# Dimitrinov74/Domain-Specific-Image-Compression

Hardware: AMD Instinct MI355X
Metric: 256x256 satellite patches encoded/s per GPU; bpp + MS-SSIM vs reference (higher is better)
Workload: dtype f32 (Winograd contractions as split-bf16 MFMA with fp32 accumulate); 1 GPU; batch=64/GPU 256x256x3 synthetic patches, modelv2 encode->decode (g_a,h_a,round,h_s,Student-t/Gaussian rate,g_s) + bpp + MS-SSIM[.3,.5,.2] on GPU + CDF tables and range coder (z,y strings) on GPU [BASELINE config 3]; global_batch=64, parallelism=per-image sharding x1, one all-reduce of 4 fp64, weights=synthetic seed 1 (checkpoints absent from the reference)

## Files before the change

domain-specific-image-compression_amd/csrc/dsic_math.h:

```cpp
#pragma once
#include <stdint.h>

#if defined(__HIPCC__)
#define DM_HD __host__ __device__ inline
#else
#define DM_HD inline
#endif

namespace dsic {
namespace dm {

#define DM_LN2_HI 6.93147180369123816490e-01
#define DM_LN2_LO 1.90821492927058770002e-10
#define DM_INV_LN2 1.44269504088896338700e+00
#define DM_SQRT2 1.41421356237309514547e+00
#define DM_INV_SQRT_PI 5.64189583547756279280e-01
#define DM_HALF_LOG_2PI 9.18938533204672780563e-01

DM_HD double from_bits(uint64_t b) {
  union {
    uint64_t u;
    double d;
  } v;
  v.u = b;
// ... 12 lines not shown
  while (k > 1000) {
    x *= 8.98846567431157953865e+307;
    k -= 1023;
  }
  while (k < -1000) {
    x *= 2.22507385850720138309e-308;
    k += 1022;
  }
  return x * from_bits((uint64_t)(k + 1023) << 52);
}

DM_HD double exp(double x) {
  if (x != x) return x;
  if (x > 709.0) return from_bits(0x7FF0000000000000ULL);
  if (x < -745.0) return 0.0;
  const double t = x * DM_INV_LN2;
  const int k = (int)(t < 0 ? t - 0.5 : t + 0.5);
  const double r = (x - (double)k * DM_LN2_HI) - (double)k * DM_LN2_LO;
  double p = 1.0 / 87178291200.0;
  p = p * r + 1.0 / 6227020800.0;
  p = p * r + 1.0 / 479001600;
  p = p * r + 1.0 / 39916800;
  p = p * r + 1.0 / 3628800;
  p = p * r + 1.0 / 362880;
  p = p * r + 1.0 / 40320;
  p = p * r + 1.0 / 5040;
  p = p * r + 1.0 / 720;
  p = p * r + 1.0 / 120;
  p = p * r + 1.0 / 24;
  p = p * r + 1.0 / 6;
  p = p * r + 0.5;
  p = p * r + 1.0;
  p = p * r + 1.0;
  return scale2(p, k);
}

DM_HD double log(double x) {
  if (x != x || x < 0) return from_bits(0x7FF8000000000000ULL);
  if (x == 0) return from_bits(0xFFF0000000000000ULL);
  int e = 0;
  if (x < 2.22507385850720138309e-308) {
    x *= 4503599627370496.0;
    e = -52;
  }
  uint64_t bits = to_bits(x);
  e += (int)((bits >> 52) & 0x7FF) - 1023;
  double m = from_bits((bits & 0x000FFFFFFFFFFFFFULL) | 0x3FF0000000000000ULL);
  if (m > DM_SQRT2) {
    m = m * 0.5;
    e += 1;
  }
  const double f = m - 1.0;
  const double s = f / (2.0 + f);
  const double z = s * s;
  double p = 1.0 / 25;
  for (int n = 11; n >= 1; --n) p = p * z + 1.0 / (double)(2 * n + 1);
  p = p * z + 1.0;
  const double de = (double)e;
  return de * DM_LN2_HI + (2.0 * s * p + de * DM_LN2_LO);
}

DM_HD double lgamma(double x) {
  double acc = 1.0;
  while (x < 12.0) {
    acc = acc * x;
    x = x + 1.0;
  }
  const double xi = 1.0 / x, x2 = xi * xi;
  double ser = 1.0 / 156;
  ser = ser * x2 - 691.0 / 360360;
  ser = ser * x2 + 1.0 / 1188;
  ser = ser * x2 - 1.0 / 1680;
  ser = ser * x2 + 1.0 / 1260;
  ser = ser * x2 - 1.0 / 360;
  ser = ser * x2 + 1.0 / 12;
  const double st = (x - 0.5) * log(x) - x + DM_HALF_LOG_2PI + ser * xi;
  return st - log(acc);
}

DM_HD double erfc_pos(double u) {
  if (u < 1.5) {
    const double u2 = u * u;
    double term = u, sum = u;
    for (int n = 1; n < 200; ++n) {
      term = term * (2.0 * u2) / (double)(2 * n + 1);
      sum = sum + term;
      if (term < sum * 1e-17) break;
    }
    return 1.0 - 2.0 * DM_INV_SQRT_PI * exp(-u2) * sum;
  }
  double d = u;
  for (int n = 120; n >= 1; --n) d = u + (0.5 * (double)n) / d;
  return exp(-u * u) * DM_INV_SQRT_PI / d;
}

DM_HD double normal_cdf(double x) {
  const double u = x / DM_SQRT2;
  if (u >= 0) return 1.0 - 0.5 * erfc_pos(u);
  return 0.5 * erfc_pos(-u);
}

DM_HD double betacf(double a, double b, double x) {
  const double TINY = 1e-300;
  const double qab = a + b, qap = a + 1.0, qam = a - 1.0;
  double c = 1.0, d = 1.0 - qab * x / qap;
  if (d < TINY && d > -TINY) d = TINY;
  d = 1.0 / d;
  double h = d;
  for (int m = 1; m <= 400; ++m) {
    const double dm_ = (double)m, m2 = 2.0 * dm_;
    double aa = dm_ * (b - dm_) * x / ((qam + m2) * (a + m2));
    d = 1.0 + aa * d;
    if (d < TINY && d > -TINY) d = TINY;
    c = 1.0 + aa / c;
    if (c < TINY && c > -TINY) c = TINY;
    d = 1.0 / d;
    h = h * d * c;
    aa = -(a + dm_) * (qab + dm_) * x / ((a + m2) * (qap + m2));
    d = 1.0 + aa * d;
    if (d < TINY && d > -TINY) d = TINY;
    c = 1.0 + aa / c;
    if (c < TINY && c > -TINY) c = TINY;
    d = 1.0 / d;
    const double del = d * c;
    h = h * del;
    double dev = del - 1.0;
    if (dev < 0) dev = -dev;
    if (dev < 3e-16) break;
  }
  return h;
}

DM_HD double betainc(double a, double b, double x, double xc) {
  if (x <= 0.0) return 0.0;
  if (xc <= 0.0) return 1.0;
  const double lbeta = lgamma(a + b) - lgamma(a) - lgamma(b);
  const double front = exp(lbeta + a * log(x) + b * log(xc));
  if (x < (a + 1.0) / (a + b + 2.0)) return front * betacf(a, b, x) / a;
  return 1.0 - front * betacf(b, a, xc) / b;
}

DM_HD double student_t_tail(double t, double nu) {
  const double t2 = t * t;
  const double den = nu + t2;
  const double x = nu / den, xc = t2 / den;
  return 0.5 * betainc(0.5 * nu, 0.5, x, xc);
}

DM_HD double student_t_cdf(double t, double nu) {
  const double tail = student_t_tail(t, nu);
  return t > 0 ? 1.0 - tail : tail;
}


DM_HD double erf_pos(double u) {
  if (u < 1.5) {
    const double u2 = u * u;
    double term = u, sum = u;
    for (int n = 1; n < 200; ++n) {
      term = term * (2.0 * u2) / (double)(2 * n + 1);
      sum = sum + term;
      if (term < sum * 1e-17) break;
    }
    return 2.0 * DM_INV_SQRT_PI * exp(-u2) * sum;
  }
  if (u > 6.0) return 1.0;
  return 1.0 - erfc_pos(u);
}

DM_HD float erff_rn(float a) {
  const double u = (double)a;
  if (u != u) return a;
  return u < 0 ? -(float)erf_pos(-u) : (float)erf_pos(u);
}

DM_HD float gaussian_cdf_f32(float x) {
  const float a = x / 1.41421354f;
  const float e = erff_rn(a);
  const float s = 1.0f + e;
  return 0.5f * s;
}

DM_HD float sum_f32_torch(const float* p, int n) {
  float a0 = 0.0f, a1 = 0.0f, a2 = 0.0f, a3 = 0.0f;
  int i = 0;
  while (i + 16 <= n) {
    for (int j = 0; j < 16; ++j, ++i) a0 = a0 + p[i];
    a1 = a1 + a0;
    a0 = 0.0f;
    if ((i & 0xF0) == 0) {
      a2 = a2 + a1;
      a1 = 0.0f;
      if ((i & 0xF00) == 0) {
        a3 = a3 + a2;
        a2 = 0.0f;
      }
    }
  }
  for (; i < n; ++i) a0 = a0 + p[i];
  a0 = a0 + a1;
  a0 = a0 + a2;
  a0 = a0 + a3;
  return a0;
}

DM_HD void finish_table(const float* F, int L, uint16_t* out, float* pmf, uint16_t* raw) {
  for (int k = 0; k < L; ++k) {
    float p = F[k + 1] - F[k];
    if (p < 1e-12f) p = 1e-12f;
    pmf[k] = p;
  }
  const float total = sum_f32_torch(pmf, L);
  double cum = 0.0;
  uint32_t u16 = 0;
  for (int k = 0; k < L; ++k) {
    out[k] = (uint16_t)((uint32_t)(((uint64_t)u16 * (uint64_t)(65536 - L)) / 65535u) + (uint32_t)k);
    if (raw) raw[k] = (uint16_t)u16;
    const float q = pmf[k] / total;
    cum = cum + (double)q;
    float c = (float)cum;
    if (k == L - 1 && c < 1.0f) c = 1.0f;
    float sc = c * 65535.0f;
    if (sc < 0.0f) sc = 0.0f;
    if (sc > 65535.0f) sc = 65535.0f;
    u16 = (uint32_t)sc;
  }
  if (raw) raw[L] = (uint16_t)u16;
}

DM_HD float boundary_f32(int smin, int k) { return (float)(smin + k) - 0.5f; }
DM_HD float table_cdf_gauss(int smin, int k, float sigma) {
  return gaussian_cdf_f32(boundary_f32(smin, k) / sigma);
}
DM_HD float table_cdf_student(int smin, int k, float sigma, float nu) {
  return (float)student_t_cdf((double)boundary_f32(smin, k) / (double)sigma, (double)nu);
}

}
}
```

domain-specific-image-compression_amd/csrc/entropy.hip:

```cpp
#include "common.h"
#include "dsic_math.h"

#include <climits>

namespace dsic {

__global__ __launch_bounds__(256) void support_kernel(const float* __restrict__ y,
                                                      const float* __restrict__ z,
                                                      int* __restrict__ meta, int64_t ny, int64_t nz,
                                                      int tail) {
  __shared__ float red[2][4];
  __shared__ int bad_any;
  const int b = blockIdx.x;
  for (int which = 0; which < 2; ++which) {
    const float* p = which ? z + (size_t)b * nz : y + (size_t)b * ny;
    const int64_t n = which ? nz : ny;
    float mn = p[0], mx = p[0];
    bool bad = false;
    for (int64_t i = threadIdx.x; i < n; i += 256) {
      const float v = p[i];
      bad |= !(fabsf(v) < 1.0e9f);
      mn = fminf(mn, v);
      mx = fmaxf(mx, v);
    }
#pragma unroll
    for (int o = 32; o > 0; o >>= 1) {
      mn = fminf(mn, __shfl_down(mn, o, 64));
      mx = fmaxf(mx, __shfl_down(mx, o, 64));
    }
    if (threadIdx.x == 0) bad_any = 0;
    __syncthreads();
    if ((threadIdx.x & 63) == 0) {
      red[0][threadIdx.x >> 6] = mn;
      red[1][threadIdx.x >> 6] = mx;
    }
    if (__any(bad) && (threadIdx.x & 63) == 0) atomicOr(&bad_any, 1);
    __syncthreads();
    if (threadIdx.x == 0) {
      mn = fminf(fminf(red[0][0], red[0][1]), fminf(red[0][2], red[0][3]));
      mx = fmaxf(fmaxf(red[1][0], red[1][1]), fmaxf(red[1][2], red[1][3]));
      if (bad_any) {
        meta[4 * b + 2 * which] = 0;
        meta[4 * b + 2 * which + 1] = 0;
      } else {
        const int lo = (int)floorf(mn) - tail, hi = (int)ceilf(mx) + tail;
        meta[4 * b + 2 * which] = lo;
        meta[4 * b + 2 * which + 1] = hi - lo + 1;
      }
    }
    __syncthreads();
  }
}

__device__ __forceinline__ void finish_table_wave(float* F, int L, uint16_t* out, float* pmf, int lane) {
  for (int k = lane; k < L; k += 64) {
    float p = F[k + 1] - F[k];
    if (p < 1e-12f) p = 1e-12f;
    pmf[k] = p;
  }
  __builtin_amdgcn_s_waitcnt(0xc07f);
  __builtin_amdgcn_wave_barrier();
  const float total = dm::sum_f32_torch(pmf, L);
  double cum = 0.0;
  for (int base = 0; base < L; base += 64) {
    const int k = base + lane;
    const float q = k < L ? pmf[k] / total : 0.0f;
    const int n = L - base < 64 ? L - base : 64;
    float mine = 0.0f;
    for (int j = 0; j < n; ++j) {
      const float qj = __builtin_bit_cast(float, __builtin_amdgcn_readlane(__builtin_bit_cast(int, q), j));
      cum = cum + (double)qj;
      float c = (float)cum;
      if (base + j == L - 1 && c < 1.0f) c = 1.0f;
      if (j == lane) mine = c;
    }
    if (k < L) F[k] = mine;
  }
  __builtin_amdgcn_s_waitcnt(0xc07f);
  __builtin_amdgcn_wave_barrier();
  for (int k = lane; k < L; k += 64) {
    uint32_t u16 = 0;
    if (k > 0) {
      float sc = F[k - 1] * 65535.0f;
      if (sc < 0.0f) sc = 0.0f;
      if (sc > 65535.0f) sc = 65535.0f;
      u16 = (uint32_t)sc;
    }
    out[k] = (uint16_t)((u16 * (uint32_t)(65536 - L)) / 65535u + (uint32_t)k);
  }
}

template <bool STUDENT>
__global__ __launch_bounds__(256) void tables_kernel(const float* __restrict__ sigma,
                                                     const float* __restrict__ nu, int sb,
                                                     const int* __restrict__ meta, int meta_off,
                                                     uint16_t* __restrict__ tables, int C, int Lmax,
                                                     int ntables, int* __restrict__ err) {
  extern __shared__ float shm[];
  const int wave = threadIdx.x >> 6, lane = threadIdx.x & 63;
  const int tid = blockIdx.x * 4 + wave;
  if (tid >= ntables) return;
  const int b = tid / C, c = tid % C;
  const int smin = meta[4 * b + meta_off], L = meta[4 * b + meta_off + 1];
  if (L > Lmax || L < 1) {
    if (lane == 0) atomicOr(err, 1);
    return;
  }
  float* F = shm + (size_t)wave * (2 * Lmax + 1);
  float* pmf = F + Lmax + 1;
  const float sg = sigma[(size_t)b * sb + c];
  const float nv = STUDENT ? nu[(size_t)b * sb + c] : 0.0f;
  if (STUDENT && smin <= 0 && smin + L >= 1) {
    const int whi = smin + L > 1 - smin ? smin + L : 1 - smin;
    for (int w = 1 + lane; w <= whi; w += 64) {
      const double tail = dm::student_t_tail((double)((float)w - 0.5f) / (double)sg, (double)nv);
      if (w <= smin + L) F[w - smin] = (float)(1.0 - tail);
      if (1 - w >= smin) F[1 - w - smin] = (float)tail;
    }
  } else {
    for (int k = lane; k <= L; k += 64)
      F[k] = STUDENT ? dm::table_cdf_student(smin, k, sg, nv) : dm::table_cdf_gauss(smin, k, sg);
  }
  __builtin_amdgcn_s_waitcnt(0xc07f);
  __builtin_amdgcn_wave_barrier();
  finish_table_wave(F, L, tables + ((size_t)b * C + c) * Lmax, pmf, lane);
}

constexpr int ZT_IMGS = 16;

__global__ __launch_bounds__(256) void gauss_tables_kernel(const float* __restrict__ sigma,
                                                           const int* __restrict__ meta,
                                                           uint16_t* __restrict__ tables, int B, int C, int Lmax,
                                                           int rowmax, int* __restrict__ err) {
  extern __shared__ float shm[];
  __shared__ int ulo, uhi;
  const int wave = threadIdx.x >> 6, lane = threadIdx.x & 63;
  const int c = blockIdx.x, b0 = blockIdx.y * ZT_IMGS;
  const int b1 = B - b0 < ZT_IMGS ? B : b0 + ZT_IMGS;
  const float sg = sigma[c];
  if (wave == 0) {
    int lo = INT_MAX, hi = INT_MIN;
    if (b0 + lane < b1 && lane < ZT_IMGS) {
      const int smin = meta[4 * (b0 + lane) + 2], L = meta[4 * (b0 + lane) + 3];
      if (L >= 1 && L <= Lmax) {
        lo = smin;
        hi = smin + L;
      }
    }
#pragma unroll
    for (int o = 32; o > 0; o >>= 1) {
      lo = min(lo, __shfl_xor(lo, o, 64));
      hi = max(hi, __shfl_xor(hi, o, 64));
    }
    if (lane == 0) {
      ulo = lo;
      uhi = hi;
    }
  }
  __syncthreads();
  const int lo = ulo, hi = uhi;
  const bool shared_row = hi >= lo && (int64_t)hi - lo < (int64_t)rowmax;
  float* row = shm;
  if (shared_row)
    for (int u = lo + (int)threadIdx.x; u <= hi; u += 256) row[u - lo] = dm::table_cdf_gauss(u, 0, sg);
  __syncthreads();
  float* F = shm + rowmax + (size_t)wave * (2 * Lmax + 1);
  float* pmf = F + Lmax + 1;
  for (int b = b0 + wave; b < b1; b += 4) {
    const int smin = meta[4 * b + 2], L = meta[4 * b + 3];
    if (L > Lmax || L < 1) {
      if (lane == 0) atomicOr(err, 1);
      continue;
    }
    for (int k = lane; k <= L; k += 64) F[k] = shared_row ? row[smin + k - lo] : dm::table_cdf_gauss(smin, k, sg);
    __builtin_amdgcn_s_waitcnt(0xc07f);
    __builtin_amdgcn_wave_barrier();
    finish_table_wave(F, L, tables + ((size_t)b * C + c) * Lmax, pmf, lane);
    __builtin_amdgcn_s_waitcnt(0xc07f);
    __builtin_amdgcn_wave_barrier();
  }
}

__device__ __forceinline__ void put_bits(uint32_t* out32, int64_t cap_bits, int64_t off, uint32_t v,
                                         int len, int* overflow) {
  if (off + len > cap_bits) {
    *overflow = 1;
    return;
  }
  const int64_t w = off >> 5;
  const int s = (int)(off & 31), space = 32 - s;
  if (len <= space) {
    atomicOr(out32 + w, __builtin_bswap32(v << (space - len)));
  } else {
    const int rest = len - space;
    atomicOr(out32 + w, __builtin_bswap32(v >> rest));
    atomicOr(out32 + w + 1, __builtin_bswap32(v << (32 - rest)));
  }
}

__device__ __forceinline__ void put_ones(uint32_t* out32, int64_t cap_bits, int64_t off, uint32_t count,
                                         int* overflow) {
  while (count > 0) {
    const int len = count > 32 ? 32 : (int)count;
    put_bits(out32, cap_bits, off, len == 32 ? 0xFFFFFFFFu : ((1u << len) - 1u), len, overflow);
    off += len;
    count -= len;
  }
}

constexpr int PLACE_WIN = 512;
__device__ __forceinline__ void or_word(uint32_t* out32, uint32_t* win, int64_t wbase, int64_t w, uint32_t v) {
  const int64_t i = w - wbase;
  if (i >= 0 && i < PLACE_WIN) atomicOr(win + i, v);
  else atomicOr(out32 + w, v);
}

__device__ __forceinline__ void put_bits_w(uint32_t* out32, uint32_t* win, int64_t wbase, int64_t cap_bits,
                                           int64_t off, uint32_t v, int len, int* overflow) {
  if (off + len > cap_bits) {
    *overflow = 1;
    return;
  }
  const int64_t w = off >> 5;
  const int s = (int)(off & 31), space = 32 - s;
  if (len <= space) {
    or_word(out32, win, wbase, w, __builtin_bswap32(v << (space - len)));
  } else {
    const int rest = len - space;
    or_word(out32, win, wbase, w, __builtin_bswap32(v >> rest));
    or_word(out32, win, wbase, w + 1, __builtin_bswap32(v << (32 - rest)));
  }
}

__device__ __forceinline__ void put_ones_w(uint32_t* out32, uint32_t* win, int64_t wbase, int64_t cap_bits,
                                           int64_t off, uint32_t count, int* overflow) {
  while (count > 0) {
    const int len = count > 32 ? 32 : (int)count;
    put_bits_w(out32, win, wbase, cap_bits, off, len == 32 ? 0xFFFFFFFFu : ((1u << len) - 1u), len, overflow);
    off += len;
    count -= len;
  }
}

#ifndef ENC_SELECT
#define ENC_SELECT 1
#endif
template <int J>
__device__ __forceinline__ void wlane(uint32_t& rec, uint32_t v) {
  asm volatile("v_writelane_b32 %0, %1, %2" : "+v"(rec) : "s"(v), "n"(J));
}

template <int J>
__device__ __forceinline__ uint32_t rlane(uint32_t v) {
  uint32_t r;
  asm volatile("v_readlane_b32 %0, %1, %2" : "=s"(r) : "v"(v), "n"(J));
  return r;
}

template <int J>
__device__ __forceinline__ void enc_step(uint32_t& low, uint32_t& lowm1, uint32_t& span, uint32_t& cl,
                                         uint32_t& ch, uint32_t clo16, uint32_t chi16, uint32_t& rec_low,
                                         uint32_t& rec_high) {
  const uint32_t cl_next = J < 63 ? rlane<(J < 63 ? J + 1 : 63)>(clo16) : 0u;
  const uint32_t ch_next = J < 63 ? rlane<(J < 63 ? J + 1 : 63)>(chi16) : 0u;
  uint32_t lo_add, hi_add;
#if ENC_SELECT
  {
    const uint32_t ml = __umulhi(span, cl), mh = __umulhi(span, ch);
    lo_add = span ? ml : cl;
    hi_add = span ? mh : ch;
  }
#else
  if (__builtin_expect(span == 0u, 0)) {
    lo_add = cl;
    hi_add = ch;
  } else {
    lo_add = __umulhi(span, cl);
    hi_add = __umulhi(span, ch);
  }
#endif
  const uint32_t low1 = low + lo_add;
  const uint32_t high1 = lowm1 + hi_add;
  const uint32_t span1 = hi_add - lo_add;
  wlane<J>(rec_low, low1);
  wlane<J>(rec_high, high1);
  const int nb = __builtin_clz(low1 ^ high1);
  const uint32_t q2 = (high1 | ~low1) << 1;
  const int m = __builtin_clz(q2 << nb);
  const int sh = nb + m;
  span = span1 << sh;
  low = (low1 << sh) & 0x7FFFFFFFu;
  lowm1 = low - 1u;
  cl = cl_next;
  ch = ch_next;
}

template <int J0>
__device__ __forceinline__ void enc_steps8(uint32_t& low, uint32_t& lowm1, uint32_t& span, uint32_t& cl,
                                           uint32_t& ch, uint32_t clo16, uint32_t chi16, uint32_t& rec_low,
                                           uint32_t& rec_high) {
  enc_step<J0 + 0>(low, lowm1, span, cl, ch, clo16, chi16, rec_low, rec_high);
  enc_step<J0 + 1>(low, lowm1, span, cl, ch, clo16, chi16, rec_low, rec_high);
  enc_step<J0 + 2>(low, lowm1, span, cl, ch, clo16, chi16, rec_low, rec_high);
  enc_step<J0 + 3>(low, lowm1, span, cl, ch, clo16, chi16, rec_low, rec_high);
  enc_step<J0 + 4>(low, lowm1, span, cl, ch, clo16, chi16, rec_low, rec_high);
  enc_step<J0 + 5>(low, lowm1, span, cl, ch, clo16, chi16, rec_low, rec_high);
  enc_step<J0 + 6>(low, lowm1, span, cl, ch, clo16, chi16, rec_low, rec_high);
  enc_step<J0 + 7>(low, lowm1, span, cl, ch, clo16, chi16, rec_low, rec_high);
}

__global__ __launch_bounds__(1024) void range_encode_kernel(
    const float* __restrict__ y, const float* __restrict__ z, const int* __restrict__ meta,
    const uint16_t* __restrict__ tab_y, const uint16_t* __restrict__ tab_z, int Lmax, int M, int HWy,
    int N, int HWz, uint8_t* __restrict__ out, int64_t cap_y, int64_t cap_z,
    int* __restrict__ lengths, int* __restrict__ err, int nstreams, int per_element_y) {
  const int lane = threadIdx.x & 63;
  const int sid = __builtin_amdgcn_readfirstlane(blockIdx.x * (blockDim.x >> 6) + (threadIdx.x >> 6));
  if (sid >= nstreams) return;
  const int nimg = nstreams >> 1;
  const int which = sid < nimg ? 1 : 0, b = which ? sid : sid - nimg;
  const int C = which ? M : N, HW = which ? HWy : HWz;
  const int64_t n = (int64_t)C * HW;
  const float* sym = which ? y + (size_t)b * n : z + (size_t)b * n;
  const bool per_element = which && per_element_y;
  const uint16_t* tab = (which ? tab_y + (size_t)b * (per_element ? (size_t)M * HWy : (size_t)M) * Lmax
                               : tab_z + (size_t)b * N * Lmax);
  const int smin = meta[4 * b + (which ? 0 : 2)], L = meta[4 * b + (which ? 1 : 3)];
  const int64_t stride = cap_z + cap_y;
  uint32_t* dst32 = (uint32_t*)(out + (size_t)b * stride + (which ? cap_z : 0));
  const int64_t cap_bits = (which ? cap_y : cap_z) * 8;
  if (L > Lmax || L < 1) {
    if (lane == 0) {
// ... 562 lines not shown
    int64_t rw = 0;
    for (int64_t g = 0; g < n; ++g) {
      const uint32_t d = value - low;
      const uint32_t bound = span ? __umulhi(span, ck16) : ck16;
      const int hits = __popcll(__ballot(bound <= d) & valid);
      const uint32_t lo_add = __builtin_amdgcn_readlane(bound, hits - 1);
      const uint32_t hi_mul = __builtin_amdgcn_readlane(bound, hits & 63);
      const uint32_t hi_add = hits == L ? span : hi_mul;
      {
        const int sv = hits - 1 + smin;
        const int ln = (int)(g & 63);
        asm volatile("s_mov_b32 m0, %2\n\ts_nop 3\n\tv_writelane_b32 %0, %1, m0" : "+v"(outv) : "s"(sv), "s"(ln));
        if (ln == 63) dst[g - 63 + lane] = (float)outv;
      }
      const uint32_t low1 = low + lo_add;
      const uint32_t high1 = lowm1 + hi_add;
      const uint32_t span1 = hi_add - lo_add;
      const int nb = __builtin_clz(low1 ^ high1);
      const uint32_t q2 = (high1 | ~low1) << 1;
      const int m = __builtin_clz(q2 << nb);
      const int sh = nb + m;
      if (__builtin_expect(sh < 32, 1)) {
        span = span1 << sh;
        low = (low1 << sh) & 0x7FFFFFFFu;
        const uint32_t v2 = sh ? ((value << sh) | take(sh)) : value;
        value = m ? (v2 ^ 0x80000000u) : v2;
      } else {
        uint32_t lo2 = low1 << nb, hi2 = (high1 << nb) | ((1u << nb) - 1u);
        value = nb ? ((value << nb) | take(nb)) : value;
        lo2 = (lo2 << m) & 0x7FFFFFFFu;
        hi2 = (hi2 << m) | 0x80000000u | ((1u << m) - 1u);
        value = ((value << m) | take(m)) ^ 0x80000000u;
        low = lo2;
        span = hi2 - lo2 + 1u;
      }
      lowm1 = low - 1u;
      if (++in_r == HW) {
        in_r = 0;
        rw += 1;
        ck16 = ck16_next;
        if (rw + 1 < C) ck16_next = load_row16(rw + 1);
      }
    }
    if (n & 63) {
      const int64_t g0 = n & ~(int64_t)63;
      if (lane < (int)(n & 63)) dst[g0 + lane] = (float)outv;
    }
    return;
  }
  int64_t row = 0;
  int in_row = 0;
  auto load_seg = [&](const uint16_t* t, int seg) -> uint32_t {
    const int k = seg * 64 + lane;
    return k < L ? (uint32_t)t[k] : 0x10000u;
  };
  uint32_t ck0 = load_seg(gt, 0);
  for (int64_t g = 0; g < n; ++g) {
    {
      const uint16_t* t = gt + (size_t)row * Lmax;
      const bool new_row = per_element || in_row + 1 == HW;
      uint32_t ck0_next = ck0;
      if (new_row && g + 1 < n) ck0_next = load_seg(gt + (size_t)(row + 1) * Lmax, 0);
      const uint32_t d = value - low;
      const uint32_t r = high - low;
      int cnt = 0;
      uint32_t c_low = 0, c_high = 0x10000u, carry_low = 0;
      bool carry = false;
      for (int seg = 0; seg < nseg; ++seg) {
        const int k = seg * 64 + lane;
        const uint32_t ck = seg == 0 ? ck0 : load_seg(t, seg);
        const uint32_t bound = (uint32_t)(((uint64_t)r * ck + ck) >> 16);
        const int hits = __popcll(__ballot(k < L && bound <= d));
        if (hits == 0) {
          if (carry) {
            c_low = carry_low;
            c_high = __builtin_amdgcn_readlane(ck, 0);
          }
          break;
        }
        cnt += hits;
        if (hits < 64) {
          c_low = __builtin_amdgcn_readlane(ck, hits - 1);
          c_high = __builtin_amdgcn_readlane(ck, hits);
          break;
        }
        carry = true;
        carry_low = __builtin_amdgcn_readlane(ck, 63);
        if (seg + 1 == nseg) {
          c_low = carry_low;
          c_high = 0x10000u;
        }
      }
      ck0 = ck0_next;
      if (new_row) {
        row += 1;
        in_row = 0;
      } else {
        in_row += 1;
      }
      const int sidx = cnt - 1;
      if (lane == 0) dst[g] = (float)(sidx + smin);
      const uint32_t hi_add = (uint32_t)(((uint64_t)r * c_high + c_high) >> 16);
      const uint32_t lo_add = (uint32_t)(((uint64_t)r * c_low + c_low) >> 16);
      high = (low - 1u) + hi_add;
      low = low + lo_add;
      const int nb = __builtin_clz(low ^ high);
      low <<= nb;
      high = (high << nb) | ((1u << nb) - 1u);
      value = nb ? ((value << nb) | take(nb)) : value;
      const uint32_t e3 = (low << 1) & ~(high << 1);
      const int m = __builtin_clz(~e3);
      low = (low << m) & 0x7FFFFFFFu;
      high = (high << m) | 0x80000000u | ((1u << m) - 1u);
      value = m ? (((value << m) | take(m)) ^ 0x80000000u) : value;
    }
  }
}

}

using namespace dsic;

#ifndef ENC_ABL
#define ENC_ABL 0
#endif
#if ENC_ABL
__device__ int enc_abl_err_sink;
static int* abl_err(int* err) {
  void* p = nullptr;
  return hipGetSymbolAddress(&p, HIP_SYMBOL(enc_abl_err_sink)) == hipSuccess ? (int*)p : err;
}
#else
static int* abl_err(int* err) { return err; }
#endif


extern "C" int dsic_latent_support(const float* y_nchw, const float* z_nchw, int* meta, int B,
                                   int64_t n_y, int64_t n_z, int tail, void* stream) {
  DSIC_REQUIRE(y_nchw && z_nchw && meta, "latent_support: null pointer");
  DSIC_REQUIRE(B > 0 && n_y > 0 && n_z > 0 && tail >= 0, "latent_support: bad argument");
  if (ENC_ABL & 1) return DSIC_OK;
  hipLaunchKernelGGL(support_kernel, dim3(B), dim3(256), 0, (hipStream_t)stream, y_nchw, z_nchw, meta,
                     n_y, n_z, tail);
  return check_launch("latent_support");
}

static int tables_launch(bool student, const float* sigma, const float* nu, int per_image,
                         const int* meta, int meta_off, uint16_t* tables, int B, int C, int Lmax,
                         int* err, hipStream_t st) {
  DSIC_REQUIRE(sigma && meta && tables && err && (!student || nu), "cdf_tables: null pointer");
  DSIC_REQUIRE(B > 0 && C > 0 && Lmax >= 1 && Lmax <= 1000, "cdf_tables: Lmax=%d must be in [1,1000]", Lmax);
  if (ENC_ABL & 2) return DSIC_OK;
  err = abl_err(err);
  const int ntables = B * C;
  const size_t shm = (size_t)4 * (2 * Lmax + 1) * sizeof(float);
  const int sb = per_image ? C : 0;
  if (student) {
    hipLaunchKernelGGL(tables_kernel<true>, dim3(ceil_div(ntables, 4)), dim3(256), shm, st, sigma, nu, sb,
                       meta, meta_off, tables, C, Lmax, ntables, err);
  } else if (sb == 0) {
    const int rowmax = 4 * Lmax;
    hipLaunchKernelGGL(gauss_tables_kernel, dim3(C, ceil_div(B, ZT_IMGS)), dim3(256), shm + rowmax * sizeof(float),
                       st, sigma, meta, tables, B, C, Lmax, rowmax, err);
  } else {
    hipLaunchKernelGGL(tables_kernel<false>, dim3(ceil_div(ntables, 4)), dim3(256), shm, st, sigma, nu, sb,
                       meta, meta_off, tables, C, Lmax, ntables, err);
  }
  return check_launch("cdf_tables");
}

extern "C" int dsic_cdf_tables_gauss(const float* sigma_z, const int* meta, uint16_t* tables, int B,
                                     int N, int Lmax, int* err, void* stream) {
  return tables_launch(false, sigma_z, nullptr, 0, meta, 2, tables, B, N, Lmax, err, (hipStream_t)stream);
}

extern "C" int dsic_cdf_tables_student(const float* sigma, const float* nu, const int* meta,
                                       uint16_t* tables, int B, int rows, int Lmax, int* err,
                                       void* stream) {
  return tables_launch(true, sigma, nu, 1, meta, 0, tables, B, rows, Lmax, err, (hipStream_t)stream);
}

extern "C" int dsic_range_encode(const float* y_nchw, const float* z_nchw, const int* meta,
                                 const uint16_t* tab_y, const uint16_t* tab_z, int Lmax, int B, int M,
                                 int HWy, int N, int HWz, uint8_t* out, int64_t cap_y, int64_t cap_z,
                                 int* lengths, int* err, int streams_per_wg, int per_element_y,
                                 void* stream) {
  DSIC_REQUIRE(y_nchw && z_nchw && meta && tab_y && tab_z && out && lengths && err,
               "range_encode: null pointer");
  DSIC_REQUIRE(B > 0 && M > 0 && N > 0 && HWy > 0 && HWz > 0, "range_encode: empty latent");
  DSIC_REQUIRE(cap_y % 4 == 0 && cap_z % 4 == 0 && cap_y >= 8 && cap_z >= 8,
               "range_encode: capacities must be multiples of 4 and >= 8");
  DSIC_REQUIRE(streams_per_wg >= 1 && streams_per_wg <= 16, "range_encode: streams_per_wg must be in [1,16]");
  hipLaunchKernelGGL(range_encode_kernel, dim3(ceil_div(2 * B, streams_per_wg)), dim3(64 * streams_per_wg), 0,
                     (hipStream_t)stream,
                     y_nchw, z_nchw, meta, tab_y, tab_z, Lmax, M, HWy, N, HWz, out, cap_y, cap_z, lengths,
                     err, 2 * B, per_element_y ? 1 : 0);
  return check_launch("range_encode");
}

static int64_t place_records(int B, int64_t ny, int64_t nz) {
  int gy, ky, gz, kz;
  place_slicing(ny, gy, ky);
  place_slicing(nz, gz, kz);
  return (int64_t)B * (ky + kz);
}

extern "C" int64_t dsic_range_encode_workspace_size(int B, int M, int HWy, int N, int HWz) {
  if (B <= 0 || M <= 0 || HWy <= 0 || N <= 0 || HWz <= 0) return -1;
  const int64_t ny = (int64_t)M * HWy, nz = (int64_t)N * HWz;
  const int64_t total = (int64_t)B * (ny + nz);
  return 12 * total + 8 * (int64_t)B + 8 + 8 * place_records(B, ny, nz);
}

extern "C" int dsic_range_encode_ws(const float* y_nchw, const float* z_nchw, const int* meta,
                                    const uint16_t* tab_y, const uint16_t* tab_z, int Lmax, int B, int M,
                                    int HWy, int N, int HWz, uint8_t* out, int64_t cap_y, int64_t cap_z,
                                    int* lengths, int* err, int per_element_y, void* workspace,
                                    int64_t workspace_bytes, void* stream) {
  DSIC_REQUIRE(y_nchw && z_nchw && meta && tab_y && tab_z && out && lengths && err && workspace,
               "range_encode_ws: null pointer");
  DSIC_REQUIRE(B > 0 && M > 0 && N > 0 && HWy > 0 && HWz > 0, "range_encode_ws: empty latent");
  DSIC_REQUIRE(cap_y % 4 == 0 && cap_z % 4 == 0 && cap_y >= 8 && cap_z >= 8,
               "range_encode_ws: capacities must be multiples of 4 and >= 8");
  DSIC_REQUIRE(workspace_bytes >= dsic_range_encode_workspace_size(B, M, HWy, N, HWz),
               "range_encode_ws: workspace too small");
  err = abl_err(err);
  SplitGeom G;
  G.B = B; G.M = M; G.HWy = HWy; G.N = N; G.HWz = HWz; G.Lmax = Lmax; G.per_element_y = per_element_y ? 1 : 0;
  G.ny = (int64_t)M * HWy;
  G.nz = (int64_t)N * HWz;
  DSIC_REQUIRE(G.ny < ((int64_t)1 << 29) && G.nz < ((int64_t)1 << 29), "range_encode_ws: string too long");
  place_slicing(G.ny, G.gy, G.ky);
  place_slicing(G.nz, G.gz, G.kz);
  const int64_t nslices = (int64_t)B * (G.ky + G.kz);
  DSIC_REQUIRE(nslices < ((int64_t)1 << 30), "range_encode_ws: too many strings");
  const int64_t total = (int64_t)B * (G.ny + G.nz);
  uint32_t* pairs = (uint32_t*)workspace;
  uint32_t* rec_low = pairs + total;
  uint32_t* rec_high = rec_low + total;
  uint32_t* final_low = rec_high + total;
  uint2* slices = (uint2*)(((uintptr_t)(final_low + 2 * B) + 7) & ~(uintptr_t)7);
  hipStream_t st = (hipStream_t)stream;
  int rc = DSIC_OK;
  if (!(ENC_ABL & 4)) {
    const int64_t nmax = G.ny > G.nz ? G.ny : G.nz;
    const int gx = (int)((nmax + 255) / 256 < 256 ? (nmax + 255) / 256 : 256);
    hipLaunchKernelGGL(enc_pack_kernel, dim3(gx, 2 * B), dim3(256), 0, st, y_nchw, z_nchw, meta, tab_y, tab_z, G,
                       pairs, err);
    rc = check_launch("range_encode_ws: pack");
    if (rc != DSIC_OK) return rc;
  }
  if (!(ENC_ABL & 16)) {
    hipLaunchKernelGGL(enc_chain_kernel, dim3(2 * B), dim3(64), 0, st, pairs, meta, G, rec_low, rec_high, final_low);
    rc = check_launch("range_encode_ws: chain");
    if (rc != DSIC_OK) return rc;
  }
  if (!(ENC_ABL & 8)) {
    const int nwg = (int)((nslices + PLACE_WAVES - 1) / PLACE_WAVES);
    hipLaunchKernelGGL(enc_place_sum_kernel, dim3(nwg), dim3(64 * PLACE_WAVES), 0, st, meta, G, rec_low, rec_high,
                       slices);
    rc = check_launch("range_encode_ws: place summarize");
    if (rc != DSIC_OK) return rc;
    hipLaunchKernelGGL(enc_place_emit_kernel, dim3(nwg), dim3(64 * PLACE_WAVES), 0, st, meta, G, rec_low, rec_high,
                       slices, final_low, out, cap_y, cap_z, lengths, err);
    rc = check_launch("range_encode_ws: place emit");
  }
  return rc;
}

extern "C" int dsic_range_decode(const uint8_t* in, int64_t stride, const int* lengths, int lstride,
                                 int loff, const int* meta, int meta_off, const uint16_t* tables,
                                 int Lmax, int B, int C, int HW, int per_element, float* out_nchw,
                                 int* err, void* stream) {
  DSIC_REQUIRE(in && lengths && meta && tables && out_nchw && err, "range_decode: null pointer");
  DSIC_REQUIRE(B > 0 && C > 0 && HW > 0 && Lmax >= 1, "range_decode: bad argument");
  DSIC_REQUIRE(meta_off == 0 || meta_off == 2, "range_decode: meta_off must be 0 (y) or 2 (z)");
  DSIC_REQUIRE(stride % 4 == 0, "range_decode: stride must be a multiple of 4");
  hipLaunchKernelGGL(range_decode_kernel, dim3(B), dim3(64), 0, (hipStream_t)stream, in, stride,
                     lengths, lstride, loff, meta, meta_off, tables, Lmax, C, HW, out_nchw, err, B, per_element ? 1 : 0);
  return check_launch("range_decode");
}

extern "C" int dsic_stream_create_masked(const uint32_t* mask_host, int words, void** stream_out) {
  DSIC_REQUIRE(mask_host && stream_out && words >= 1, "stream_create_masked: bad argument");
  hipStream_t st = nullptr;
  hipError_t e = hipExtStreamCreateWithCUMask(&st, (uint32_t)words, mask_host);
  if (e != hipSuccess) {
    set_error("hipExtStreamCreateWithCUMask: %s", hipGetErrorString(e));
    return DSIC_EHIP;
  }
  *stream_out = (void*)st;
  return DSIC_OK;
}
extern "C" int dsic_stream_destroy(void* stream) {
  hipError_t e = hipStreamDestroy((hipStream_t)stream);
  if (e != hipSuccess) {
    set_error("hipStreamDestroy: %s", hipGetErrorString(e));
    return DSIC_EHIP;
  }
  return DSIC_OK;
}

extern "C" double dsic_host_normal_cdf(double x) { return dm::normal_cdf(x); }
extern "C" double dsic_host_student_t_cdf(double t, double nu) { return dm::student_t_cdf(t, nu); }
extern "C" float dsic_host_gaussian_cdf_f32(float x) { return dm::gaussian_cdf_f32(x); }
extern "C" float dsic_host_exp_f32(float x) { return (float)dm::exp((double)x); }
extern "C" int dsic_host_pmf_to_uint16_cdf(const float* pmf_host, int L, int C, uint16_t* out_host) {
  DSIC_REQUIRE(pmf_host && out_host && L >= 1 && C >= 1, "host_pmf_to_uint16_cdf: bad argument");
  for (int c = 0; c < C; ++c) {
    double cum = 0.0;
    out_host[c] = 0;
    for (int k = 0; k < L; ++k) {
      cum = cum + (double)pmf_host[(size_t)k * C + c];
      float v = (float)cum;
      if (k == L - 1 && v < 1.0f) v = 1.0f;
      float sc = v * 65535.0f;
      if (sc < 0.0f) sc = 0.0f;
      if (sc > 65535.0f) sc = 65535.0f;
// ... 15 lines not shown
```

Baseline: 11540 images/s.

## Pack multiple CDF tables per wave and flatten boundary evaluation across lanes

The CDF-table kernels now assign several tables to each wavefront, three for the Student-t/per-image path and two for the Gaussian z path. Boundary CDF evaluations are flattened across all tables in the group so lanes stay busy when individual tables are short, and the scan and finish steps interleave the tables to amortise the serial readlane prefix loop. The pmf buffer is dropped in favour of in-place reuse of F, and betainc is evaluated through a single betacf call with selected arguments to reduce divergence. The risks are higher register pressure (launch bounds now 256,7), more LDS per block, and more complex indexing.

```diff
diff --git a/domain-specific-image-compression_amd/csrc/dsic_math.h b/domain-specific-image-compression_amd/csrc/dsic_math.h
--- a/domain-specific-image-compression_amd/csrc/dsic_math.h
+++ b/domain-specific-image-compression_amd/csrc/dsic_math.h
@@ -188,6 +188,23 @@
   return t > 0 ? 1.0 - tail : tail;
 }
 
+DM_HD double betainc_onepass(double a, double b, double x, double xc) {
+  if (x <= 0.0) return 0.0;
+  if (xc <= 0.0) return 1.0;
+  const double lbeta = lgamma(a + b) - lgamma(a) - lgamma(b);
+  const double front = exp(lbeta + a * log(x) + b * log(xc));
+  const bool lower = x < (a + 1.0) / (a + b + 2.0);
+  const double h = betacf(lower ? a : b, lower ? b : a, lower ? x : xc);
+  return lower ? front * h / a : 1.0 - front * h / b;
+}
+
+DM_HD double student_t_tail_onepass(double t, double nu) {
+  const double t2 = t * t;
+  const double den = nu + t2;
+  const double x = nu / den, xc = t2 / den;
+  return 0.5 * betainc_onepass(0.5 * nu, 0.5, x, xc);
+}
+
 
 DM_HD double erf_pos(double u) {
   if (u < 1.5) {
diff --git a/domain-specific-image-compression_amd/csrc/entropy.hip b/domain-specific-image-compression_amd/csrc/entropy.hip
--- a/domain-specific-image-compression_amd/csrc/entropy.hip
+++ b/domain-specific-image-compression_amd/csrc/entropy.hip
@@ -52,81 +52,181 @@
   }
 }
 
-__device__ __forceinline__ void finish_table_wave(float* F, int L, uint16_t* out, float* pmf, int lane) {
-  for (int k = lane; k < L; k += 64) {
-    float p = F[k + 1] - F[k];
-    if (p < 1e-12f) p = 1e-12f;
-    pmf[k] = p;
-  }
+__device__ __forceinline__ void wave_lds_sync() {
   __builtin_amdgcn_s_waitcnt(0xc07f);
   __builtin_amdgcn_wave_barrier();
-  const float total = dm::sum_f32_torch(pmf, L);
-  double cum = 0.0;
-  for (int base = 0; base < L; base += 64) {
+}
+
+template <int G>
+__device__ __forceinline__ void finish_tables_wave(float* const (&F)[G], const int (&L)[G], uint16_t* const (&out)[G],
+                                                   int lane) {
+  int Lw = 0;
+#pragma unroll
+  for (int t = 0; t < G; ++t) Lw = L[t] > Lw ? L[t] : Lw;
+  for (int base = 0; base < Lw; base += 64) {
     const int k = base + lane;
-    const float q = k < L ? pmf[k] / total : 0.0f;
-    const int n = L - base < 64 ? L - base : 64;
-    float mine = 0.0f;
+    float p[G];
+#pragma unroll
+    for (int t = 0; t < G; ++t) {
+      p[t] = 0.0f;
+      if (k < L[t]) {
+        p[t] = F[t][k + 1] - F[t][k];
+        if (p[t] < 1e-12f) p[t] = 1e-12f;
+      }
+    }
+    wave_lds_sync();
+#pragma unroll
+    for (int t = 0; t < G; ++t)
+      if (k < L[t]) F[t][k] = p[t];
+    wave_lds_sync();
+  }
+  float total[G];
+  {
+    const int mine = lane % G;
+    const float* pm = F[0];
+    int n = L[0];
+#pragma unroll
+    for (int t = 1; t < G; ++t)
+      if (mine == t) {
+        pm = F[t];
+        n = L[t];
+      }
+    const float s = dm::sum_f32_torch(pm, n);
+#pragma unroll
+    for (int t = 0; t < G; ++t) total[t] = __builtin_bit_cast(float, __builtin_amdgcn_readlane(__builtin_bit_cast(int, s), t));
+  }
+  double cum[G];
+#pragma unroll
+  for (int t = 0; t < G; ++t) cum[t] = 0.0;
+  for (int base = 0; base < Lw; base += 64) {
+    const int k = base + lane;
+    float q[G], mine[G];
+#pragma unroll
+    for (int t = 0; t < G; ++t) {
+      q[t] = k < L[t] ? F[t][k] / total[t] : 0.0f;
+      mine[t] = 0.0f;
+    }
+    const int n = Lw - base < 64 ? Lw - base : 64;
     for (int j = 0; j < n; ++j) {
-      const float qj = __builtin_bit_cast(float, __builtin_amdgcn_readlane(__builtin_bit_cast(int, q), j));
-      cum = cum + (double)qj;
-      float c = (float)cum;
-      if (base + j == L - 1 && c < 1.0f) c = 1.0f;
-      if (j == lane) mine = c;
-    }
-    if (k < L) F[k] = mine;
-  }
-  __builtin_amdgcn_s_waitcnt(0xc07f);
-  __builtin_amdgcn_wave_barrier();
-  for (int k = lane; k < L; k += 64) {
-    uint32_t u16 = 0;
-    if (k > 0) {
-      float sc = F[k - 1] * 65535.0f;
-      if (sc < 0.0f) sc = 0.0f;
-      if (sc > 65535.0f) sc = 65535.0f;
-      u16 = (uint32_t)sc;
-    }
-    out[k] = (uint16_t)((u16 * (uint32_t)(65536 - L)) / 65535u + (uint32_t)k);
-  }
-}
+#pragma unroll
+      for (int t = 0; t < G; ++t) {
+        const float qj = __builtin_bit_cast(float, __builtin_amdgcn_readlane(__builtin_bit_cast(int, q[t]), j));
+        cum[t] = cum[t] + (double)qj;
+        if (j == lane) mine[t] = (float)cum[t];
+      }
+    }
+#pragma unroll
+    for (int t = 0; t < G; ++t) {
+      if (k < L[t]) {
+        float c = mine[t];
+        if (k == L[t] - 1 && c < 1.0f) c = 1.0f;
+        F[t][k] = c;
+      }
+    }
+  }
+  wave_lds_sync();
+#pragma unroll
+  for (int t = 0; t < G; ++t) {
+    for (int k = lane; k < L[t]; k += 64) {
+      uint32_t u16 = 0;
+      if (k > 0) {
+        float sc = F[t][k - 1] * 65535.0f;
+        if (sc < 0.0f) sc = 0.0f;
+        if (sc > 65535.0f) sc = 65535.0f;
+        u16 = (uint32_t)sc;
+      }
+      out[t][k] = (uint16_t)((u16 * (uint32_t)(65536 - L[t])) / 65535u + (uint32_t)k);
+    }
+  }
+}
+
+constexpr int TABLES_PER_WAVE = 3;
 
 template <bool STUDENT>
-__global__ __launch_bounds__(256) void tables_kernel(const float* __restrict__ sigma,
+__global__ __launch_bounds__(256, 7) void tables_kernel(const float* __restrict__ sigma,
                                                      const float* __restrict__ nu, int sb,
                                                      const int* __restrict__ meta, int meta_off,
                                                      uint16_t* __restrict__ tables, int C, int Lmax,
                                                      int ntables, int* __restrict__ err) {
+  constexpr int G = TABLES_PER_WAVE;
   extern __shared__ float shm[];
-  const int wave = threadIdx.x >> 6, lane = threadIdx.x & 63;
-  const int tid = blockIdx.x * 4 + wave;
-  if (tid >= ntables) return;
-  const int b = tid / C, c = tid % C;
-  const int smin = meta[4 * b + meta_off], L = meta[4 * b + meta_off + 1];
-  if (L > Lmax || L < 1) {
-    if (lane == 0) atomicOr(err, 1);
-    return;
-  }
-  float* F = shm + (size_t)wave * (2 * Lmax + 1);
-  float* pmf = F + Lmax + 1;
-  const float sg = sigma[(size_t)b * sb + c];
-  const float nv = STUDENT ? nu[(size_t)b * sb + c] : 0.0f;
-  if (STUDENT && smin <= 0 && smin + L >= 1) {
-    const int whi = smin + L > 1 - smin ? smin + L : 1 - smin;
-    for (int w = 1 + lane; w <= whi; w += 64) {
-      const double tail = dm::student_t_tail((double)((float)w - 0.5f) / (double)sg, (double)nv);
-      if (w <= smin + L) F[w - smin] = (float)(1.0 - tail);
-      if (1 - w >= smin) F[1 - w - smin] = (float)tail;
-    }
-  } else {
-    for (int k = lane; k <= L; k += 64)
-      F[k] = STUDENT ? dm::table_cdf_student(smin, k, sg, nv) : dm::table_cdf_gauss(smin, k, sg);
-  }
-  __builtin_amdgcn_s_waitcnt(0xc07f);
-  __builtin_amdgcn_wave_barrier();
-  finish_table_wave(F, L, tables + ((size_t)b * C + c) * Lmax, pmf, lane);
+  const int wave = __builtin_amdgcn_readfirstlane(threadIdx.x >> 6), lane = threadIdx.x & 63;
+  const int t0 = (blockIdx.x * 4 + wave) * G;
+  if (t0 >= ntables) return;
+  float* F[G];
+  uint16_t* out[G];
+  int L[G], smin[G], first[G], row[G];
+  bool straddle[G];
+  int total = 0;
+#pragma unroll
+  for (int t = 0; t < G; ++t) {
+    const int tid = t0 + t;
+    F[t] = shm + ((size_t)wave * G + t) * (Lmax + 1);
+    out[t] = tables + (size_t)tid * Lmax;
+    L[t] = 0;
+    smin[t] = 0;
+    row[t] = 0;
+    straddle[t] = false;
+    first[t] = total;
+    if (tid < ntables) {
+      const int b = tid / C, c = tid % C;
+      const int s = meta[4 * b + meta_off], l = meta[4 * b + meta_off + 1];
+      if (l > Lmax || l < 1) {
+        if (lane == 0) atomicOr(err, 1);
+      } else {
+        L[t] = l;
+        smin[t] = s;
+        row[t] = b * sb + c;
+        straddle[t] = STUDENT && s <= 0 && s + l >= 1;
+        total += straddle[t] ? (s + l > 1 - s ? s + l : 1 - s) : l + 1;
+      }
+    }
+  }
+  for (int i = lane; i < total; i += 64) {
+    int t = 0;
+#pragma unroll
+    for (int tt = 1; tt < G; ++tt)
+      if (i >= first[tt]) t = tt;
+    int sm = smin[0], l = L[0], r = row[0], j = i - first[0];
+    bool st = straddle[0];
+    float* Ft = F[0];
+#pragma unroll
+    for (int tt = 1; tt < G; ++tt)
+      if (t == tt) {
+        sm = smin[tt];
+        l = L[tt];
+        r = row[tt];
+        j = i - first[tt];
+        st = straddle[tt];
+        Ft = F[tt];
+      }
+    const float sg = sigma[r];
+    if (STUDENT) {
+      const float nv = nu[r];
+      const int w = 1 + j;
+      const double tq = (double)((float)(st ? w : sm + j) - 0.5f) / (double)sg;
+      const double tail = dm::student_t_tail_onepass(tq, (double)nv);
+      int ipos = -1, ineg = -1;
+      if (st) {
+        if (w <= sm + l) ipos = w - sm;
+        if (1 - w >= sm) ineg = 1 - w - sm;
+      } else if (tq > 0) {
+        ipos = j;
+      } else {
+        ineg = j;
+      }
+      if (ipos >= 0) Ft[ipos] = (float)(1.0 - tail);
+      if (ineg >= 0) Ft[ineg] = (float)tail;
+    } else {
+      Ft[j] = dm::table_cdf_gauss(sm, j, sg);
+    }
+  }
+  wave_lds_sync();
+  finish_tables_wave<G>(F, L, out, lane);
 }
 
 constexpr int ZT_IMGS = 16;
+constexpr int ZT_PAIR = 2;
 
 __global__ __launch_bounds__(256) void gauss_tables_kernel(const float* __restrict__ sigma,
                                                            const int* __restrict__ meta,
@@ -134,7 +234,7 @@
                                                            int rowmax, int* __restrict__ err) {
   extern __shared__ float shm[];
   __shared__ int ulo, uhi;
-  const int wave = threadIdx.x >> 6, lane = threadIdx.x & 63;
+  const int wave = __builtin_amdgcn_readfirstlane(threadIdx.x >> 6), lane = threadIdx.x & 63;
   const int c = blockIdx.x, b0 = blockIdx.y * ZT_IMGS;
   const int b1 = B - b0 < ZT_IMGS ? B : b0 + ZT_IMGS;
   const float sg = sigma[c];
@@ -164,20 +264,43 @@
   if (shared_row)
     for (int u = lo + (int)threadIdx.x; u <= hi; u += 256) row[u - lo] = dm::table_cdf_gauss(u, 0, sg);
   __syncthreads();
-  float* F = shm + rowmax + (size_t)wave * (2 * Lmax + 1);
-  float* pmf = F + Lmax + 1;
-  for (int b = b0 + wave; b < b1; b += 4) {
-    const int smin = meta[4 * b + 2], L = meta[4 * b + 3];
-    if (L > Lmax || L < 1) {
-      if (lane == 0) atomicOr(err, 1);
-      continue;
-    }
-    for (int k = lane; k <= L; k += 64) F[k] = shared_row ? row[smin + k - lo] : dm::table_cdf_gauss(smin, k, sg);
-    __builtin_amdgcn_s_waitcnt(0xc07f);
-    __builtin_amdgcn_wave_barrier();
-    finish_table_wave(F, L, tables + ((size_t)b * C + c) * Lmax, pmf, lane);
-    __builtin_amdgcn_s_waitcnt(0xc07f);
-    __builtin_amdgcn_wave_barrier();
+  float* F[ZT_PAIR];
+  uint16_t* out[ZT_PAIR];
+  int L[ZT_PAIR], smin[ZT_PAIR];
+  for (int bp = b0 + wave; bp < b1; bp += 4 * ZT_PAIR) {
+#pragma unroll
+    for (int t = 0; t < ZT_PAIR; ++t) {
+      const int b = bp + 4 * t;
+      F[t] = shm + rowmax + ((size_t)wave * ZT_PAIR + t) * (Lmax + 1);
+      out[t] = tables + ((size_t)b * C + c) * Lmax;
+      L[t] = 0;
+      smin[t] = 0;
+      if (b < b1) {
+        const int s = meta[4 * b + 2], l = meta[4 * b + 3];
+        if (l > Lmax || l < 1) {
+          if (lane == 0) atomicOr(err, 1);
+        } else {
+          L[t] = l;
+          smin[t] = s;
+        }
+      }
+    }
+    if (shared_row) {
+#pragma unroll
+      for (int t = 0; t < ZT_PAIR; ++t)
+        for (int k = lane; k <= L[t] && L[t] > 0; k += 64) F[t][k] = row[smin[t] + k - lo];
+    } else {
+      const int total = (L[0] > 0 ? L[0] + 1 : 0) + (L[1] > 0 ? L[1] + 1 : 0);
+      const int first1 = L[0] > 0 ? L[0] + 1 : 0;
+      for (int i = lane; i < total; i += 64) {
+        const int t = i >= first1 ? 1 : 0;
+        const int k = t ? i - first1 : i;
+        F[t][k] = dm::table_cdf_gauss(smin[t], k, sg);
+      }
+    }
+    wave_lds_sync();
+    finish_tables_wave<ZT_PAIR>(F, L, out, lane);
+    wave_lds_sync();
   }
 }
 
@@ -1046,18 +1169,21 @@
   DSIC_REQUIRE(B > 0 && C > 0 && Lmax >= 1 && Lmax <= 1000, "cdf_tables: Lmax=%d must be in [1,1000]", Lmax);
   if (ENC_ABL & 2) return DSIC_OK;
   err = abl_err(err);
+  DSIC_REQUIRE((int64_t)B * C <= INT_MAX, "cdf_tables: %d x %d tables", B, C);
   const int ntables = B * C;
-  const size_t shm = (size_t)4 * (2 * Lmax + 1) * sizeof(float);
   const int sb = per_image ? C : 0;
+  const size_t shm = (size_t)4 * TABLES_PER_WAVE * (Lmax + 1) * sizeof(float);
+  const int ngroups = ceil_div(ceil_div(ntables, TABLES_PER_WAVE), 4);
   if (student) {
-    hipLaunchKernelGGL(tables_kernel<true>, dim3(ceil_div(ntables, 4)), dim3(256), shm, st, sigma, nu, sb,
+    hipLaunchKernelGGL(tables_kernel<true>, dim3(ngroups), dim3(256), shm, st, sigma, nu, sb,
                        meta, meta_off, tables, C, Lmax, ntables, err);
   } else if (sb == 0) {
     const int rowmax = 4 * Lmax;
-    hipLaunchKernelGGL(gauss_tables_kernel, dim3(C, ceil_div(B, ZT_IMGS)), dim3(256), shm + rowmax * sizeof(float),
+    const size_t zshm = (size_t)4 * ZT_PAIR * (Lmax + 1) * sizeof(float) + rowmax * sizeof(float);
+    hipLaunchKernelGGL(gauss_tables_kernel, dim3(C, ceil_div(B, ZT_IMGS)), dim3(256), zshm,
                        st, sigma, meta, tables, B, C, Lmax, rowmax, err);
   } else {
-    hipLaunchKernelGGL(tables_kernel<false>, dim3(ceil_div(ntables, 4)), dim3(256), shm, st, sigma, nu, sb,
+    hipLaunchKernelGGL(tables_kernel<false>, dim3(ngroups), dim3(256), shm, st, sigma, nu, sb,
                        meta, meta_off, tables, C, Lmax, ntables, err);
   }
   return check_launch("cdf_tables");
```

New measurement: 11560 images/s (median of 4 runs). About the same (+0.1%).
